# Lillthorin/YoloLite-Official-Repo

Hardware: AMD Instinct MI355X
Metric: images/sec (higher is better)
Workload: dtype f32

## Files before the change

### yololite-official-repo_amd/csrc/yl_convc.hip

```cpp
#include "yl_lp.h"
#if YL_BF16
#define yl_conv_dwc_kernel YL_LP_NAME(yl_conv_dwc_kernel)
#define yl_launch_conv_dwc YL_LP_NAME(yl_launch_conv_dwc)
#define yl_convc_init YL_LP_NAME(yl_convc_init)
#define yl_conv_pwt_kernel YL_LP_NAME(yl_conv_pwt_kernel)
#define yl_launch_conv_pwt YL_LP_NAME(yl_launch_conv_pwt)
#define yl_launch_conv_pwt_multi YL_LP_NAME(yl_launch_conv_pwt_multi)
#define yl_conv_dwt_kernel YL_LP_NAME(yl_conv_dwt_kernel)
#define yl_launch_conv_dwt YL_LP_NAME(yl_launch_conv_dwt)
#define yl_conv_dwk_kernel YL_LP_NAME(yl_conv_dwk_kernel)
#define yl_conv_dwl_kernel YL_LP_NAME(yl_conv_dwl_kernel)
#define yl_launch_conv_dwk YL_LP_NAME(yl_launch_conv_dwk)
#define yl_conv_dws_kernel YL_LP_NAME(yl_conv_dws_kernel)
#define yl_launch_conv_dws YL_LP_NAME(yl_launch_conv_dws)
#define yl_conv_wino_kernel YL_LP_NAME(yl_conv_wino_kernel)
#define yl_launch_conv_wino YL_LP_NAME(yl_launch_conv_wino)
#define yl_conv_kxk_kernel YL_LP_NAME(yl_conv_kxk_kernel)
#define yl_launch_conv_kxk YL_LP_NAME(yl_launch_conv_kxk)
#define yl_conv_pws_kernel YL_LP_NAME(yl_conv_pws_kernel)
#define yl_launch_conv_pws YL_LP_NAME(yl_launch_conv_pws)
#define yl_ir_kernel YL_LP_NAME(yl_ir_kernel)
#define yl_launch_conv_ir YL_LP_NAME(yl_launch_conv_ir)
#define yl_ir_supported YL_LP_NAME(yl_ir_supported)
#endif
// ... 1102 lines not shown

hipError_t yl_launch_conv_kxk(const YlConvP& p, hipStream_t st) {
  if (p.k != 3 || p.dw_k > 0 || (p.N & 3) || p.dec_boxes || p.C1 > 0 || p.w3p) return hipErrorNotSupported;
  static const int nwtab[4] = {0, 4, 8, -1};
  const int NWsel = nwtab[YL_DEV_KXK_NW(p.dev)];
  const int MTsel = (p.dev & YL_DEV_KXK_MT2) ? 2 : 1;
  if (p.NTtot == 4) {
    if (YlKxkLds::image_bytes(p.TK, 4) <= YlKxkLds::LIMIT || NWsel < 0) return hipErrorNotSupported;
    return NWsel == 8 ? kxk_go(p, 4, 1, 8, 1, st) : kxk_go(p, 4, 2, 4, 1, st);
  }
  if (p.NTtot % 7 != 0) return hipErrorNotSupported;
  if (YlKxkLds::image_bytes(p.TK, 7) <= YlKxkLds::LIMIT) return hipErrorNotSupported;
  const int gy = p.NTtot / 7;
  const bool eight = NWsel ? NWsel == 8 : ((long)p.M / 128) * gy >= 2 * 2 * YL_NUM_CU;
  return eight ? kxk_go(p, 7, 1, 8, gy, st) : kxk_go(p, 7, MTsel, 4, gy, st);
}

struct YlPwsLds {
  static constexpr size_t LIMIT = 64 * 1024;
  static constexpr int CH = 2;
  static constexpr __host__ __device__ size_t bytes(int NTA) { return (size_t)2 * CH * NTA * 1024; }
};

template <int NT, int NW, bool SC = false, bool DEC = false, int NT2 = 0>
__global__ __launch_bounds__(NW * 64, NW == 4 ? 3 : 4) void yl_conv_pws_kernel(YlConvP p) {
  constexpr int CH = YlPwsLds::CH;
  constexpr int NTA = NT + NT2;
  extern __shared__ __attribute__((aligned(16))) float yl_clds[];
  const int tid = threadIdx.x, lane = tid & 63;
  const int wave = __builtin_amdgcn_readfirstlane(tid >> 6);
  const int kq = lane >> 4, pl = lane & 15;
  const int KB = p.KB, NTtot = p.NTtot, Cin = p.Cin, M = p.M;
  const yl_act_t* const xin = p.x;
  f32x4* wl = reinterpret_cast<f32x4*>(yl_clds);
  const f32x4* wg = reinterpret_cast<const f32x4*>(p.wp);
  const int NC = (KB + CH - 1) / CH;
  const int G = (NTtot + NT - 1) / NT;
  const int bx = blockIdx.x, gx = gridDim.x;
  const YlBandSplit ws = yl_band_split(bx, gx, p.ntiles, G);
  const int per = ws.per, slot = ws.slot, band0 = ws.band0, bt = ws.bt, nmine = ws.nmine;
  const long total_chunks = (long)nmine * NC;
  auto load_chunk = [&](int g, int c, int buf) {
    for (int i = wave; i < CH * NTA; i += NW) {
      const int j = i / NTA, nt = i - j * NTA;
      int kb = c * CH + j;
      kb = kb < KB ? kb : KB - 1;
      if (NT2 > 0 && nt >= NT) {
        yl_glds16(reinterpret_cast<const f32x4*>(p.w3p) + ((size_t)kb * NT2 + (nt - NT)) * 64 + lane, wl + ((size_t)buf * CH * NTA + i) * 64);
        continue;
      }
      int ntg = g * NT + nt;
      ntg = ntg < NTtot ? ntg : NTtot - 1;
      yl_glds16(wg + ((size_t)kb * NTtot + ntg) * 64 + lane, wl + ((size_t)buf * CH * NTA + i) * 64);
    }
  };
  if (total_chunks > 0) load_chunk(slot / bt, 0, 0);
  long gchunk = 0;
  __syncthreads();
  const bool pre_add = (p.res || p.up) && p.act == YL_ACT_NONE;
  const float lo = yl_act_lo(p.act), hi = yl_act_hi(p.act);
  const int ohw = p.OH * p.OW;

  for (int wi = 0; wi < nmine; ++wi) {
    const int item = slot + wi * per;
    const int g = item / bt;
    const int nt0 = g * NT;
    const int tile = band0 + item - g * bt;
    YlPix px[1];
    {
      size_t lin = ((size_t)tile * NW + wave) * 16 + pl;
      px[0].valid = lin < (size_t)M;
      if (!px[0].valid) lin = (size_t)M - 1;
      px[0].lin = lin;
      px[0].b = 0; px[0].oy = 0; px[0].ox = 0;
      if (SC || DEC || p.up) {
        const int b = (int)(lin / ohw);
        const int rem = (int)(lin - (size_t)b * ohw);
        px[0].b = b;
        px[0].oy = rem / p.OW;
        px[0].ox = rem - px[0].oy * p.OW;
      }
    }
    const yl_act_t* xrow = xin + px[0].lin * Cin + 4 * kq;
    const float* srow = SC ? p.scale + (size_t)px[0].b * Cin + 4 * kq : nullptr;
    f32x4 acc[1][NTA];
#pragma unroll
    for (int nt = 0; nt < NTA; ++nt) acc[0][nt] = (f32x4){0.f, 0.f, 0.f, 0.f};
    if (pre_add) {
      const size_t obase = px[0].lin * p.N;
      size_t up_off = 0;
      if (p.up) {
        const int uy = (px[0].oy * p.UH) / p.OH, ux = (px[0].ox * p.UW) / p.OW;
        up_off = (((size_t)px[0].b * p.UH + uy) * p.UW + ux) * p.N;
      }
#pragma unroll
      for (int nt = 0; nt < NT; ++nt) {
        const int n = (nt0 + nt) * 16 + 4 * kq;
        if (n < p.N) {
          if (p.res) acc[0][nt] = yl_ld4(p.res + obase + n);
          if (p.up) acc[0][nt] += yl_ld4(p.up + up_off + n);
        }
      }
    }
    auto fetch = [&](int kb) {
      const bool ok = kb * 16 + 4 * kq < Cin;
      f32x4 v = yl_ld4(ok ? xrow + kb * 16 : p.zeros);
      if (SC) v *= yl_ld4(ok ? srow + kb * 16 : reinterpret_cast<const float*>(p.zeros));
      return v;
    };
    constexpr int PF = 4;
    f32x4 xr[PF];
#pragma unroll
    for (int i = 0; i < PF; ++i) xr[i] = fetch(i < KB ? i : KB - 1);
    auto chunk = [&](auto par, int c) {
      constexpr int P = decltype(par)::value;
      const int buf = (int)(gchunk & 1);
      if (gchunk + 1 < total_chunks) {
        if (c + 1 < NC) load_chunk(g, c + 1, buf ^ 1);
        else load_chunk((item + per) / bt, 0, buf ^ 1);
      }
      const f32x4* wb = wl + (size_t)buf * CH * NTA * 64 + lane;
#pragma unroll
      for (int j = 0; j < CH; ++j) {
        constexpr int dummy = 0; (void)dummy;
        const int kb = c * CH + j;
        if (kb < KB) {
          const int slot = (P * CH + j) % PF;
          constexpr int H0 = NTA > 7 ? (NTA + 1) / 2 : NTA;
          constexpr int H1 = NTA - H0;
          f32x4 xs[1] = {xr[slot]};
          xr[slot] = fetch(kb + PF < KB ? kb + PF : KB - 1);
          {
            f32x4 wq[H0], a0[1][H0];
#pragma unroll
            for (int nt = 0; nt < H0; ++nt) { wq[nt] = wb[(j * NTA + nt) * 64]; a0[0][nt] = acc[0][nt]; }
            yl_mma_step<H0, 1>(wq, xs, a0);
#pragma unroll
            for (int nt = 0; nt < H0; ++nt) acc[0][nt] = a0[0][nt];
          }
          if (H1 > 0) {
            constexpr int H1s = H1 > 0 ? H1 : 1;
            f32x4 wq[H1s], a1[1][H1s];
#pragma unroll
            for (int nt = 0; nt < H1; ++nt) { wq[nt] = wb[(j * NTA + H0 + nt) * 64]; a1[0][nt] = acc[0][H0 + nt]; }
            yl_mma_step<H1s, 1>(wq, xs, a1);
#pragma unroll
            for (int nt = 0; nt < H1; ++nt) acc[0][H0 + nt] = a1[0][nt];
          }
        }
      }
      __syncthreads();
      ++gchunk;
    };
    for (int c = 0; c < NC; c += 2) {
      chunk(std::integral_constant<int, 0>{}, c);
      if (c + 1 < NC) chunk(std::integral_constant<int, 1>{}, c + 1);
    }
    if (DEC) {
      if (NT2 > 0) {
        constexpr int N2 = NT2 > 0 ? NT2 : 1;
        f32x4 ad[1][NT], am[1][N2];
#pragma unroll
        for (int nt = 0; nt < NT; ++nt) ad[0][nt] = acc[0][nt];
#pragma unroll
        for (int nt = 0; nt < NT2; ++nt) am[0][nt] = acc[0][NT + nt];
        YlConvP pm = p;
        pm.bias = p.b3; pm.N = p.C3;
        yl_epi_fast<N2, 1>(pm, am, px, 0, kq, lo, hi, true);
        yl_epi_decode<NT, 1, false, true>(p, ad, px, 0, kq, lane);
      } else {
        yl_epi_decode<NT, 1, false, true>(p, *reinterpret_cast<f32x4 (*)[1][NT]>(&acc), px, 0, kq, lane);
      }
      continue;
    }
    if (!pre_add && (p.res || p.up || YL_SMOOTH(p.act))) yl_epi_generic<NTA, 1>(p, acc, px, nt0, kq);
    else yl_epi_fast<NTA, 1>(p, acc, px, nt0, kq, lo, hi, true);
  }
}

#define YL_PWS_NTS(X) X(13) X(11) X(9) X(8) X(7) X(6)
#define YL_PWS_NT_VALUE(NT) NT,
#define YL_PWS_NT_KERNELS(NT) \
  {{yl_conv_pws_kernel<NT, 4>, yl_conv_pws_kernel<NT, 4, true>}, {yl_conv_pws_kernel<NT, 8>, yl_conv_pws_kernel<NT, 8, true>}},
static const int pws_nts[6] = {YL_PWS_NTS(YL_PWS_NT_VALUE)};
static const YlConvKernel pws_kernels[6][2][2] = {YL_PWS_NTS(YL_PWS_NT_KERNELS)};
static const YlConvKernel pws_dec_kernels[2][2] = {{yl_conv_pws_kernel<6, 4, false, true>, yl_conv_pws_kernel<6, 4, false, true, 2>},
                                                   {yl_conv_pws_kernel<6, 8, false, true>, yl_conv_pws_kernel<6, 8, false, true, 2>}};

static hipError_t pws_go(const YlConvP& p0, hipStream_t st, int cand, bool eight) {
  const int NT = pws_nts[cand], NW = eight ? 8 : 4;
  YlConvP p = p0;
  p.ntiles = (int)(((long)p.M + 16 * NW - 1) / (16 * NW));
  const int gy = (p.NTtot + NT - 1) / NT;
  YlConvKernel kern = pws_kernels[cand][eight][p.scale != nullptr], asked = pws_kernels[cand][eight][0];
  int NTA = NT;
  if (p.dec_boxes) {
    if (NT != 6 || p.scale) return hipErrorNotSupported;
    kern = pws_dec_kernels[eight][p.w3p != nullptr];
    if (p.w3p) { NTA = NT + 2; asked = kern; }
  }
  const size_t lds = YlPwsLds::bytes(NTA);
  const int gx = yl_band_grid(yl_resident_blocks((const void*)asked, NW * 64, lds, 8), (long)p.ntiles * gy);
  hipLaunchKernelGGL(kern, dim3(gx), dim3(NW * 64), lds, st, p);
  return hipGetLastError();
}

hipError_t yl_launch_conv_pws(const YlConvP& p, hipStream_t st) {
  const bool dec = p.dec_boxes && !p.dec_raw;
  if (p.k != 1 || p.stride != 1 || p.dw_k > 0 || p.C1 > 0 || p.in_shift || (p.dec_boxes && !dec)) return hipErrorNotSupported;
  if (dec ? (p.NTtot != 6 || p.scale || p.res || p.up || (p.w3p && (p.C3 != 32 || YL_SMOOTH(p.act)))) : ((p.N & 3) != 0 || p.w3p)) return hipErrorNotSupported;
  if ((p.dev & YL_DEV_PWS_OFF) || p.KB < 5 || p.NTtot < 6) return hipErrorNotSupported;
  int NT = 0, cand = 0;
  double best = 1e30;
  long best_wi = 0;
  const long mt16 = ((long)p.M + 15) / 16;
  for (int i = dec ? 5 : 0; i < 6; ++i) {
    const long wi = mt16 * ((p.NTtot + pws_nts[i] - 1) / pws_nts[i]);
    const double sc = (double)((wi + 1023) / 1024) * pws_nts[i] * (wi < 1536 ? 1.25 : 1.0);
    if (sc < best) { best = sc; NT = pws_nts[i]; cand = i; best_wi = wi; }
  }
  if (best_wi < 1536) return hipErrorNotSupported;
  const int gy = (p.NTtot + NT - 1) / NT;
  const bool eight = ((long)p.M / 128) * gy >= 2 * 2 * YL_NUM_CU;
  return pws_go(p, st, cand, eight);
}

constexpr __host__ __device__ int yl_ir_pitch(int dk, int ds, int mt, int cbn) { return ((((4 * mt * cbn - 1) * ds + dk) * 16 + 7) / 64) * 64 + 56; }
constexpr __host__ __device__ int yl_ir_slab(int dk, int ds, int mt, int rbn, int cbn) { return ((4 * rbn - 1) * ds + dk) * yl_ir_pitch(dk, ds, mt, cbn); }
struct YlIrLds {
  static constexpr size_t LIMIT = 150 * 1024;
  size_t wpl, dwl, b2l, bytes;
  constexpr __host__ __device__ YlIrLds(int dk, int ds, int mt, int rbn, int cbn, int nt, int KB)
      : wpl((size_t)2 * yl_ir_slab(dk, ds, mt, rbn, cbn)), dwl(wpl + (size_t)2 * nt * 256), b2l(dwl + (size_t)KB * (dk * dk + 1) * 16),
        bytes((b2l + (size_t)KB * 16) * 4) {}
};

template <int KBI , int NT, int DK, int DS, int MT, int RBN , int CBN >
__global__ __launch_bounds__(RBN * CBN * 64, (DK == 3 && DS * MT <= 2 && KBI <= 3 && NT <= 3) ? 3 : 2) void yl_ir_kernel(YlConvP p) {
  constexpr int NWV = RBN * CBN, NTH = NWV * 64;
  constexpr int TH = 4 * RBN, TW = 4 * MT * CBN;
  constexpr int HH = (TH - 1) * DS + DK, HW = (TW - 1) * DS + DK, HN = HH * HW;
  constexpr int HMT = (HN + 15) / 16, HMW = (HMT + NWV - 1) / NWV;
  constexpr int PITCHF = yl_ir_pitch(DK, DS, MT, CBN), SLAB = yl_ir_slab(DK, DS, MT, RBN, CBN);
  extern __shared__ __attribute__((aligned(16))) float yl_clds[];
  const int tid = threadIdx.x, lane = tid & 63;
  const int wave = __builtin_amdgcn_readfirstlane(tid >> 6);
  const int kq = lane >> 4, pl = lane & 15;
  const int Cmid = p.Cin, KB = p.KB, NTtot = p.NTtot, C1 = p.C1, H = p.H, W = p.W, OH = p.OH, OW = p.OW, N = p.N;
  const YlIrLds L(DK, DS, MT, RBN, CBN, NT, KB);
  float* slab = yl_clds;
  f32x4* wpl = reinterpret_cast<f32x4*>(yl_clds + L.wpl);
  float* dwl = yl_clds + L.dwl;
  float* b2l = yl_clds + L.b2l;
  const f32x4* wg = reinterpret_cast<const f32x4*>(p.wp);
  const f32x4* w2g = reinterpret_cast<const f32x4*>(p.w2p);
  const yl_act_t* const xin = p.x;
  const yl_act_t* const up = p.up;
  {
    constexpr int T1 = DK * DK + 1;
    for (int i = tid; i < KB * T1 * 16; i += NTH) {
      const int kb = i / (T1 * 16), r = i - kb * (T1 * 16), t = r >> 4, ch = kb * 16 + (r & 15);
      dwl[i] = ch < Cmid ? (t < DK * DK ? p.dw_w[(size_t)t * Cmid + ch] : (p.dw_b ? p.dw_b[ch] : 0.0f)) : 0.0f;
    }
    for (int i = tid; i < KB * 16; i += NTH) b2l[i] = p.b2[i];
  }
  const float lo = yl_act_lo(p.act), hi = yl_act_hi(p.act);
  const float dlo = yl_act_lo(p.dw_act), dhi = yl_act_hi(p.dw_act);
  const float elo = yl_act_lo(p.act2), ehi = yl_act_hi(p.act2);
  const int dw_act = p.dw_act, act2 = p.act2;
  int h_r[HMW], h_c[HMW], h_lo[HMW];
  bool h_ok[HMW];
#pragma unroll
  for (int j = 0; j < HMW; ++j) {
    const int q = (wave + NWV * j) * 16 + pl;
    h_ok[j] = q < HN;
    const int qq = h_ok[j] ? q : 0;
    h_r[j] = qq / HW;
    h_c[j] = qq - h_r[j] * HW;
    h_lo[j] = h_r[j] * PITCHF + h_c[j] * 16 + 4 * kq;
  }
  const int rb = wave / CBN, cb = wave - rb * CBN;
  const int rbase = ((4 * rb + (pl >> 2)) * DS) * PITCHF + ((cb * 4 * MT + (pl & 3)) * DS) * 16 + 4 * kq;
  const bool pre_add = p.res != nullptr && p.act == YL_ACT_NONE;
  const int twn = OW / TW, thn = OH / TH;
  const int tiles_img = twn * thn;
  const int ntiles = p.B * tiles_img;
  int tile, tend, tstride;
  if ((gridDim.x & 7) == 0) {
    const int tpx = (ntiles + 7) >> 3;
    const int band0 = (blockIdx.x & 7) * tpx;
    tend = (band0 + tpx) < ntiles ? (band0 + tpx) : ntiles;
    tile = band0 + (blockIdx.x >> 3);
    tstride = gridDim.x >> 3;
  } else {
    tile = blockIdx.x; tend = ntiles; tstride = gridDim.x;
  }
  auto load_proj = [&](int kb, int buf) {
    for (int nt = wave; nt < NT; nt += NWV)
      yl_glds16(wg + ((size_t)kb * NTtot + (nt < NTtot ? nt : NTtot - 1)) * 64 + lane, wpl + ((size_t)buf * NT + nt) * 64);
  };
  unsigned gs = 0;
  if (tile < tend) load_proj(0, 0);
  __syncthreads();

  for (int wi = 0; tile < tend; tile += tstride, ++wi) {
    const int b = tile / tiles_img;
    const int trem = tile - b * tiles_img;
    const int tyi = trem / twn, txi = trem - tyi * twn;
    const int iy0 = tyi * TH * DS - p.dw_pad_t, ix0 = txi * TW * DS - p.dw_pad_l;
    YlPix px[MT];
#pragma unroll
    for (int mt = 0; mt < MT; ++mt) {
      px[mt].b = b;
      px[mt].oy = tyi * TH + 4 * rb + (pl >> 2);
      px[mt].ox = txi * TW + cb * 4 * MT + 4 * mt + (pl & 3);
      px[mt].valid = true;
      px[mt].lin = ((size_t)b * OH + px[mt].oy) * OW + px[mt].ox;
    }
    f32x4 xh[HMW][KBI];
    bool h_in[HMW];
    long uoff[HMW];
#pragma unroll
    for (int j = 0; j < HMW; ++j) {
      const int iy = iy0 + h_r[j], ix = ix0 + h_c[j];
      h_in[j] = h_ok[j] && iy >= 0 && iy < H && ix >= 0 && ix < W;
      uoff[j] = 0;
      if (up && h_in[j]) uoff[j] = ((((long)b * p.UH + (iy * p.UH) / H) * p.UW + (ix * p.UW) / W) * Cmid) + 4 * kq;
      const yl_act_t* src = xin + (((size_t)b * H + iy) * W + ix) * C1 + 4 * kq;
#pragma unroll
      for (int kbi = 0; kbi < KBI; ++kbi) {
        const bool ok = h_in[j] && (kbi * 16 + 4 * kq) < C1;
        xh[j][kbi] = yl_ld4(ok ? src + kbi * 16 : p.zeros);
      }
    }
    f32x4 acc[MT][NT];
#pragma unroll
    for (int mt = 0; mt < MT; ++mt)
#pragma unroll
      for (int nt = 0; nt < NT; ++nt) {
        acc[mt][nt] = (f32x4){0.f, 0.f, 0.f, 0.f};
        const int n = nt * 16 + 4 * kq;
        if (pre_add && n < N) acc[mt][nt] = yl_ld4(p.res + px[mt].lin * N + n);
      }
    f32x4 we[KBI], wn[KBI];
#pragma unroll
    for (int kbi = 0; kbi < KBI; ++kbi) wn[kbi] = w2g[((size_t)kbi * KB + 0) * 64 + lane];
    f32x4 un[HMW];
    auto load_up = [&](int kb, int j) {
      return yl_ld4((h_in[j] && kb * 16 + 4 * kq < Cmid) ? up + uoff[j] + kb * 16 : p.zeros);
    };
    if (up) {
#pragma unroll
      for (int j = 0; j < HMW; ++j) un[j] = load_up(0, j);
    }
    for (int kb = 0; kb < KB; ++kb, ++gs) {
      const int buf = (int)(gs & 1u);
#pragma unroll
      for (int kbi = 0; kbi < KBI; ++kbi) we[kbi] = wn[kbi];
      if (kb + 1 < KB) {
#pragma unroll
        for (int kbi = 0; kbi < KBI; ++kbi) wn[kbi] = w2g[((size_t)kbi * KB + kb + 1) * 64 + lane];
      }
      const f32x4 eb = yl_ld4(b2l + kb * 16 + 4 * kq);
      float* sb = slab + buf * SLAB;
#pragma unroll
      for (int j = 0; j < HMW; ++j) {
        f32x4 e[1][1] = {{{0.f, 0.f, 0.f, 0.f}}};
        if (up) e[0][0] = un[j];
#pragma unroll
        for (int kbi = 0; kbi < KBI; ++kbi) {
          const f32x4 wq1[1] = {we[kbi]};
          const f32x4 xq1[1] = {xh[j][kbi]};
          yl_mma_step<1, 1>(wq1, xq1, e);
        }
        if (up && kb + 1 < KB) un[j] = load_up(kb + 1, j);
        const f32x4 v = yl_sel4(h_in[j], yl_actc(e[0][0] + eb, act2, elo, ehi));
        if (h_ok[j]) *reinterpret_cast<f32x4*>(sb + h_lo[j]) = v;
      }
      __syncthreads();
      if (kb + 1 < KB) load_proj(kb + 1, buf ^ 1);
      else if (tile + tstride < tend) load_proj(0, buf ^ 1);
      const float* tapw = dwl + kb * ((DK * DK + 1) * 16) + 4 * kq;
      f32x4 xq[MT];
#pragma unroll
      for (int mt = 0; mt < MT; ++mt) xq[mt] = yl_ld4(tapw + DK * DK * 16);
      auto tap_row = [&](int dy) {
#pragma unroll
        for (int dx = 0; dx < DK; ++dx) {
          const f32x4 w = yl_ld4(tapw + (dy * DK + dx) * 16);
#pragma unroll
          for (int mt = 0; mt < MT; ++mt) {
            const f32x4 v = *reinterpret_cast<const f32x4*>(sb + rbase + dy * PITCHF + (dx + 4 * mt * DS) * 16);
            xq[mt].x = fmaf(v.x, w.x, xq[mt].x); xq[mt].y = fmaf(v.y, w.y, xq[mt].y);
            xq[mt].z = fmaf(v.z, w.z, xq[mt].z); xq[mt].w = fmaf(v.w, w.w, xq[mt].w);
          }
        }
      };
#pragma unroll 1
      for (int dy = 0; dy < DK; ++dy) tap_row(dy);
#pragma unroll
      for (int mt = 0; mt < MT; ++mt) xq[mt] = yl_actc(xq[mt], dw_act, dlo, dhi);
      f32x4 wq[NT];
      const f32x4* wrow = wpl + (size_t)buf * NT * 64 + lane;
#pragma unroll
      for (int nt = 0; nt < NT; ++nt) wq[nt] = wrow[nt * 64];
      yl_mma_step<NT, MT>(wq, xq, acc);
    }
    if (!pre_add && (p.res || YL_SMOOTH(p.act))) yl_epi_generic<NT, MT>(p, acc, px, 0, kq);
    else yl_epi_fast<NT, MT>(p, acc, px, 0, kq, lo, hi, true);
  }
}

template <int KBI, int NT, int DK, int DS, int MT, int RBN, int CBN>
static hipError_t ir_go(const YlConvP& p, hipStream_t st) {
  const size_t lds = YlIrLds(DK, DS, MT, RBN, CBN, NT, p.KB).bytes;
  const long ntiles = (long)p.B * (p.OH / (4 * RBN)) * (p.OW / (4 * MT * CBN));
  int gx = yl_resident_blocks((const void*)yl_ir_kernel<KBI, NT, DK, DS, MT, RBN, CBN>, RBN * CBN * 64, lds, 8);
  if (gx > ntiles) gx = (int)ntiles;
  if (gx >= 8) gx &= ~7;
  hipLaunchKernelGGL((yl_ir_kernel<KBI, NT, DK, DS, MT, RBN, CBN>), dim3(gx), dim3(RBN * CBN * 64), lds, st, p);
  return hipGetLastError();
}

#define YL_IR_SHAPES(X)                                                                                              \
  X(1, 2, 3, 2, 1, 2, 2) X(2, 2, 3, 1, 2, 2, 2) X(2, 3, 5, 2, 1, 2, 2) X(3, 3, 5, 1, 2, 2, 2) X(3, 6, 3, 2, 1, 2, 2)    \
  X(3, 3, 3, 1, 1, 2, 2) X(2, 6, 3, 1, 2, 2, 2) X(3, 6, 3, 1, 1, 2, 2)
#define YL_IR_BUCKET_LO(B) ((B) == 2 ? 0 : (B) == 3 ? 2 : (B) == 4 ? 3 : 4)

bool yl_ir_supported(int c1, int cmid, int n, int dk, int ds, int oh, int ow) {
  const int kbi = (c1 + 15) / 16, nt = (n + 15) / 16;
#define YL_IR_CHECK(A, B, C, D, E, R, S)                                                                             \
  if (kbi == A && nt <= B && nt > YL_IR_BUCKET_LO(B) && dk == C && ds == D && (oh % (4 * R)) == 0 &&                    \
      (ow % (4 * E * S)) == 0 && YlIrLds(C, D, E, R, S, B, (cmid + 15) / 16).bytes <= YlIrLds::LIMIT) return true;
  YL_IR_SHAPES(YL_IR_CHECK)
#undef YL_IR_CHECK
  return false;
}

hipError_t yl_launch_conv_ir(const YlConvP& p, hipStream_t st) {
  if (p.C1 <= 0 || p.k != 1 || p.dw_k == 0 || (p.N & 3)) return hipErrorNotSupported;
  const int kbi = (p.C1 + 15) / 16, nt = p.NTtot;
#define YL_IR_RUN(A, B, C, D, E, R, S)                                                                               \
  if (kbi == A && nt <= B && nt > YL_IR_BUCKET_LO(B) && p.dw_k == C && p.dw_stride == D && (p.OH % (4 * R)) == 0 &&     \
      (p.OW % (4 * E * S)) == 0 && YlIrLds(C, D, E, R, S, B, p.KB).bytes <= YlIrLds::LIMIT)                                 \
    return ir_go<A, B, C, D, E, R, S>(p, st);
  YL_IR_SHAPES(YL_IR_RUN)
#undef YL_IR_RUN
  return hipErrorNotSupported;
}

struct YlDwkLds {
  static constexpr size_t LIMIT = 96 * 1024;
  static constexpr __host__ __device__ int steps(int NT, int GW) { return GW == 1 ? 3 : (GW * NT <= 16 ? 2 : 1); }
  size_t dwl, bytes;
  constexpr __host__ __device__ YlDwkLds(int NT, int GW, int Cin)
      : dwl((size_t)2 * steps(NT, GW) * GW * NT * 256), bytes((dwl + yl_taps_floats(3, Cin)) * 4) {}
};

template <int NT, int GW, int NW>
__global__ __launch_bounds__(NW * 64, GW == 1 ? 3 : 2) void yl_conv_dwk_kernel(YlConvP p) {
  constexpr int S = YlDwkLds::steps(NT, GW);
  constexpr int PCS = S * GW * NT;
  extern __shared__ __attribute__((aligned(16))) float yl_clds[];
  const int tid = threadIdx.x, lane = tid & 63;
  const int wave = __builtin_amdgcn_readfirstlane(tid >> 6);
  const int kq = lane >> 4, pl = lane & 15;
  const int KB = p.KB, NTtot = p.NTtot;
  const int Cin = p.Cin, H = p.H, W = p.W, DS = p.dw_stride, pad_t = p.dw_pad_t, pad_l = p.dw_pad_l;
  const int ohw = p.OH * p.OW, OW = p.OW, M = p.M;
  const yl_act_t* const xin = p.x;
  const __amdgpu_buffer_rsrc_t xrs = __builtin_amdgcn_make_buffer_rsrc(
      const_cast<yl_act_t*>(xin), 0, (int)((long)p.B * H * W * Cin * (long)sizeof(yl_act_t)), 0x00020000);
  f32x4* wl = reinterpret_cast<f32x4*>(yl_clds);
  float* dwl = yl_clds + YlDwkLds(NT, GW, Cin).dwl;
  const f32x4* wg = reinterpret_cast<const f32x4*>(p.wp);
  const int NC = (KB + S - 1) / S;
  const int G = NTtot / (NT * GW);
  const int bx = blockIdx.x, gx = gridDim.x;
  const YlBandSplit ws = yl_band_split(bx, gx, p.ntiles, G);
  const int per = ws.per, slot = ws.slot, band0 = ws.band0, bt = ws.bt, nmine = ws.nmine;
  const long total_chunks = (long)nmine * NC;
  auto load_chunk = [&](int g, int c, int buf) {
    for (int i = wave; i < PCS; i += NW) {
      const int j = i / (GW * NT), nt = i - j * (GW * NT);
      const int kb = c * S + j;
      if (kb < KB) yl_glds16(wg + ((size_t)kb * NTtot + g * (GW * NT) + nt) * 64 + lane, wl + ((size_t)buf * PCS + i) * 64);
    }
  };
  if (total_chunks > 0) load_chunk(slot / bt, 0, 0);
  {
    const int nw = 9 * Cin;
    yl_glds_floats(p.dw_w, dwl, nw, tid, NW * 64);
    if (p.dw_b) yl_glds_floats(p.dw_b, dwl + nw, Cin, tid, NW * 64);
    else for (int i = tid; i < Cin; i += NW * 64) dwl[nw + i] = 0.0f;
  }
  long gchunk = 0;
  __syncthreads();
  const bool pre_add = (p.res || p.up) && p.act == YL_ACT_NONE;
  const float lo = yl_act_lo(p.act), hi = yl_act_hi(p.act);
  const float dlo = yl_act_lo(p.dw_act), dhi = yl_act_hi(p.dw_act);
  const int dw_act = p.dw_act;

  for (int wi = 0; wi < nmine; ++wi) {
    const int item = slot + wi * per;
    const int g = item / bt;
    const int nt0 = g * (GW * NT);
    const int tile = band0 + item - g * bt;
    YlPix px[1];
    {
      px[0] = yl_pix(((size_t)tile * NW + wave) * 16 + pl, M, ohw, OW);
    }
    f32x4 acc[GW][1][NT];
#pragma unroll
    for (int gw = 0; gw < GW; ++gw)
#pragma unroll
      for (int nt = 0; nt < NT; ++nt) acc[gw][0][nt] = (f32x4){0.f, 0.f, 0.f, 0.f};
    if (pre_add) {
      const size_t obase = px[0].lin * p.N;
      size_t up_off = 0;
      if (p.up) {
        const int uy = (px[0].oy * p.UH) / p.OH, ux = (px[0].ox * p.UW) / p.OW;
        up_off = (((size_t)px[0].b * p.UH + uy) * p.UW + ux) * p.N;
      }
#pragma unroll
      for (int gw = 0; gw < GW; ++gw)
#pragma unroll
        for (int nt = 0; nt < NT; ++nt) {
          const int n = (nt0 + gw * NT + nt) * 16 + 4 * kq;
          if (n < p.N) {
            if (p.res) acc[gw][0][nt] = yl_ld4(p.res + obase + n);
            if (p.up) acc[gw][0][nt] += yl_ld4(p.up + up_off + n);
          }
        }
    }
    unsigned tp[9];
#pragma unroll
    for (int tap = 0; tap < 9; ++tap) {
      const int iy = px[0].oy * DS - pad_t + tap / 3, ix = px[0].ox * DS - pad_l + tap % 3;
      const bool in = iy >= 0 && iy < H && ix >= 0 && ix < W;
      tp[tap] = in ? (unsigned)((((px[0].b * H + iy) * W + ix) * Cin + 4 * kq) * (int)sizeof(yl_act_t)) : 0x80000000u;
    }
    auto fetch = [&](f32x4 (&dst)[9], int kb) {
#pragma unroll
      for (int tap = 0; tap < 9; ++tap) {
#if YL_F16S
        dst[tap] = __builtin_convertvector(__builtin_bit_cast(yl_h16x4, __builtin_amdgcn_raw_buffer_load_b64(xrs, (int)tp[tap], kb * 32, 0)), f32x4);
#else
        dst[tap] = __builtin_bit_cast(f32x4, __builtin_amdgcn_raw_buffer_load_b128(xrs, (int)tp[tap], kb * 64, 0));
#endif
      }
    };
    f32x4 xt[9];
    fetch(xt, 0);
    for (int c = 0; c < NC; ++c, ++gchunk) {
      const int buf = (int)(gchunk & 1);
      if (gchunk + 1 < total_chunks) {
        if (c + 1 < NC) load_chunk(g, c + 1, buf ^ 1);
        else load_chunk((item + per) / bt, 0, buf ^ 1);
      }
      const f32x4* wb = wl + (size_t)buf * PCS * 64 + lane;
#pragma unroll
      for (int j = 0; j < S; ++j) {
        const int kb = c * S + j;
        if (kb < KB) {
          const int cc = kb * 16 + 4 * kq;
          const int cs = cc < Cin ? cc : Cin - 4;
          const float* tapw = dwl + cs;
          f32x4 xq[1];
          xq[0] = yl_ld4(tapw + 9 * Cin);
#pragma unroll
          for (int tap = 0; tap < 9; ++tap) {
            const f32x4 w = yl_ld4(tapw + tap * Cin);
            xq[0].x = fmaf(xt[tap].x, w.x, xq[0].x); xq[0].y = fmaf(xt[tap].y, w.y, xq[0].y);
            xq[0].z = fmaf(xt[tap].z, w.z, xq[0].z); xq[0].w = fmaf(xt[tap].w, w.w, xq[0].w);
          }
          xq[0] = yl_sel4(cc < Cin, yl_actc(xq[0], dw_act, dlo, dhi));
          if (kb + 1 < KB) fetch(xt, kb + 1);
#pragma unroll
          for (int gw = 0; gw < GW; ++gw) {
            f32x4 wq[NT];
#pragma unroll
            for (int nt = 0; nt < NT; ++nt) wq[nt] = wb[((j * GW + gw) * NT + nt) * 64];
            yl_mma_step<NT, 1>(wq, xq, acc[gw]);
          }
        }
      }
      __syncthreads();
    }
#pragma unroll
    for (int gw = 0; gw < GW; ++gw) {
      if (!pre_add && (p.res || p.up || YL_SMOOTH(p.act))) yl_epi_generic<NT, 1>(p, acc[gw], px, nt0 + gw * NT, kq);
      else yl_epi_fast<NT, 1>(p, acc[gw], px, nt0 + gw * NT, kq, lo, hi, true);
    }
  }
}

#define YL_DWK_SHAPES(X) X(7, 1, 4) X(7, 3, 4) X(8, 1, 4) X(8, 2, 4)
static YlConvKernel dwk_kernel_of(int NT, int GW, int NW) {
#define YL_DWK_PICK(A, B, C) if (NT == A && GW == B && NW == C) return yl_conv_dwk_kernel<A, B, C>;
  YL_DWK_SHAPES(YL_DWK_PICK)
#undef YL_DWK_PICK
  return nullptr;
}

static hipError_t dwk_go(const YlConvP& p0, hipStream_t st, int NT, int GW) {
  constexpr int NW = 4;
  const YlConvKernel kern = dwk_kernel_of(NT, GW, NW);
  if (!kern) return hipErrorNotSupported;
  YlConvP p = p0;
  p.ntiles = (int)(((long)p.M + 16 * NW - 1) / (16 * NW));
  const size_t lds = YlDwkLds(NT, GW, p.Cin).bytes;
  if (lds > YlDwkLds::LIMIT) return hipErrorNotSupported;
  const int G = p.NTtot / (NT * GW);
  const int gx = yl_band_grid(yl_resident_blocks((const void*)kern, NW * 64, lds, 8), (long)p.ntiles * G);
  hipLaunchKernelGGL(kern, dim3(gx), dim3(NW * 64), lds, st, p);
  return hipGetLastError();
}

static YlConvKernel dwl_kernel_of(int NTT);
static hipError_t dwl_go(const YlConvP& p0, hipStream_t st, YlConvKernel kern);

hipError_t yl_launch_conv_dwk(const YlConvP& p, hipStream_t st) {
  if (p.dw_k != 3 || (p.N & 3) || p.dec_boxes || p.C1 > 0 || p.KB < 12 || p.NTtot <= 8) return hipErrorNotSupported;
  if ((size_t)p.B * p.H * p.W * p.Cin * sizeof(yl_act_t) >= ((size_t)1 << 31)) return hipErrorNotSupported;
  const int sel = YL_DEV_DWK(p.dev) == 2 ? 0 : (YL_DEV_DWK(p.dev) == 1 ? 1 : 2);
  if (sel == 0) return hipErrorNotSupported;
  if (!YL_F16S && !(p.dev & YL_DEV_DWL_OFF) && p.dw_stride == 1 && p.dw_pad_t == 1 && p.dw_pad_l == 1 && !p.scale &&
      (size_t)p.B * p.H * p.W * p.Cin < ((size_t)1 << 31)) {
    const long wins = (long)p.B * ((p.OW + 7) >> 3) * ((p.OH + 7) >> 3);
    if (((long)p.B * p.OH * p.OW * 10 >= wins * 64 * 8 && wins >= 3 * YL_NUM_CU) || (p.dev & YL_DEV_DWL_ALL)) {
      if (const YlConvKernel kl = dwl_kernel_of(p.NTtot)) return dwl_go(p, st, kl);
    }
  }
  if (p.NTtot == 21) return dwk_go(p, st, 7, sel == 2 ? 3 : 1);
  if (p.NTtot == 16) return dwk_go(p, st, 8, sel == 2 ? 2 : 1);
  if (p.NTtot % 7 == 0) return dwk_go(p, st, 7, 1);
  if (p.NTtot % 8 == 0) return dwk_go(p, st, 8, 1);
  return hipErrorNotSupported;
}

struct YlDwlLds {
  static constexpr size_t LIMIT = 128 * 1024;
  static constexpr int RP = 12, RM = 512;
  int NTP;
  size_t Rl, dwl, bytes;
  constexpr __host__ __device__ YlDwlLds(int NTT, int KB)
      : NTP((NTT + 7) & ~7), Rl((size_t)3 * NTP * 64), dwl(Rl + 2 * 2 * RM), bytes(dwl * 16 + (size_t)KB * 160 * 4) {}
};

template <int NTT>
__global__ __launch_bounds__(512, 2) void yl_conv_dwl_kernel(YlConvP p) {
  constexpr YlDwlLds L(NTT, 0);
  constexpr int RP = YlDwlLds::RP, RM = YlDwlLds::RM, NTP = L.NTP;
  constexpr int NCH = NTT == 16 ? 4 : 6;
  static_assert(NTT == 16 || NTT == 21, "n-tile groups");
  auto c0of = [](int c) { return NTT == 16 ? 4 * c : (c <= 3 ? 4 * c : 12 + 3 * (c - 3)); };
  extern __shared__ __attribute__((aligned(16))) float yl_clds[];
  f32x4* const Wl = reinterpret_cast<f32x4*>(yl_clds);
  f32x4* const Rl = Wl + L.Rl;
  float* const dwl = reinterpret_cast<float*>(Wl + L.dwl);
  const int tid = threadIdx.x, lane = tid & 63;
  const int wave = __builtin_amdgcn_readfirstlane(tid >> 6);
  const int kq = lane >> 4, pl = lane & 15;
  const int KB = p.KB, NTtot = p.NTtot, Cin = p.Cin, H = p.H, W = p.W, OH = p.OH, OW = p.OW;
  const int WX = (OW + 7) >> 3, WY = (OH + 7) >> 3;
  const int wimg = WX * WY;
  const long WTOT = (long)p.B * wimg;
  const yl_act_t* const xin = p.x;
  const int wgmax = KB * NTtot - 1;
  const int bx = blockIdx.x, gx = gridDim.x;
  const YlBandSplit ws = yl_band_split(bx, gx, p.ntiles);
  const int per = ws.per, slot = ws.slot, band0 = ws.band0, band1 = ws.band1;
  const int rs = wave * 64 + lane;
  const int rP = rs >> 2, rkq = (rs & 3) ^ (((rP >> 2) & 1) << 1);
  const int ry = rP / RP, rx = rP - ry * RP;
  const bool rpix = ry < 10 && rx < 10;
  const int wsel = wave >> 2, qy = (wave >> 1) & 1, qx = wave & 1;
  const int sy = pl >> 2, sx = pl & 3;
  int ts[9];
#pragma unroll
  for (int tap = 0; tap < 9; ++tap) {
    const int P = (4 * qy + sy + tap / 3) * RP + 4 * qx + sx + tap % 3;
    ts[tap] = wsel * RM + 4 * P + (kq ^ (((P >> 2) & 1) << 1));
  }
  for (int i = tid; i < KB * 160; i += 512) {
    const int kb = i / 160, r = i - kb * 160, t = r >> 4, ch = kb * 16 + (r & 15);
    dwl[i] = ch < Cin ? (t < 9 ? p.dw_w[(size_t)t * Cin + ch] : (p.dw_b ? p.dw_b[ch] : 0.0f)) : 0.0f;
  }
  const __amdgpu_buffer_rsrc_t xrs = __builtin_amdgcn_make_buffer_rsrc(
      const_cast<yl_act_t*>(xin), 0, (int)((long)p.B * H * W * Cin * (long)sizeof(yl_act_t)), 0x00020000);
  const __amdgpu_buffer_rsrc_t wrs = __builtin_amdgcn_make_buffer_rsrc(
      const_cast<float*>(p.wp), 0, (int)((long)KB * NTtot * 1024), 0x00020000);
  constexpr unsigned OOB = 0x80000000u;
  const int lane16 = lane * 16;
  const int sh = KB & 1;
  const bool pre_add = (p.res || p.up) && p.act == YL_ACT_NONE;
  const float lo = yl_act_lo(p.act), hi = yl_act_hi(p.act);
  const float dlo = yl_act_lo(p.dw_act), dhi = yl_act_hi(p.dw_act);
  const int dw_act = p.dw_act;

  unsigned voff[2];
  auto issue_win = [&](int kb, int buf) {
#pragma unroll
    for (int w2 = 0; w2 < 2; ++w2)
      __builtin_amdgcn_raw_ptr_buffer_load_lds(xrs, (__attribute__((address_space(3))) void*)(Rl + (buf * 2 + w2) * RM + wave * 64), 16,
                                               (int)voff[w2], kb * 16 * (int)sizeof(yl_act_t), 0, 0);
  };
  auto issue_wts = [&](int kb, int wb) {
#pragma unroll
    for (int j = 0; j < NTP / 8; ++j) {
      const int i = wave + 8 * j;
      int src = kb * NTtot + (i < NTT ? i : 0);
// ... 927 lines not shown
```

Baseline: 50820.

## Software-pipeline expansion GEMM of next chunk with depthwise taps in IR kernel

Restructures the fused inverted-residual kernel so the expansion (1x1 MMA) for the next channel block, or for the next tile's first block, is computed and written to the alternate LDS slab while the depthwise taps of the current block run. The expansion work is split into per-row groups interleaved with the tap loads and FMAs using sched_barriers, and input staging, weight loads and residual preloads move one step ahead. The aim is to hide LDS and global latency and keep matrix and vector units busy at the same time. The cost is higher register pressure (tap values are held in registers, plus staged state) and more complex control flow, including an explicit waitcnt before the barrier.

```diff
diff --git a/yololite-official-repo_amd/csrc/yl_convc.hip b/yololite-official-repo_amd/csrc/yl_convc.hip
--- a/yololite-official-repo_amd/csrc/yl_convc.hip
+++ b/yololite-official-repo_amd/csrc/yl_convc.hip
@@ -1428,24 +1428,27 @@
   unsigned gs = 0;
   if (tile < tend) load_proj(0, 0);
   __syncthreads();
-
-  for (int wi = 0; tile < tend; tile += tstride, ++wi) {
-    const int b = tile / tiles_img;
-    const int trem = tile - b * tiles_img;
+  if (tile >= tend) return;
+
+  constexpr int RG = 1, NG = DK / RG;
+  f32x4 xh[HMW][KBI];
+  bool h_in[HMW];
+  long uoff[HMW];
+  f32x4 un[HMW];
+  f32x4 we[KBI], eb;
+  int etile = tile, ekb = 0;
+  auto load_up = [&](int kb, int j) __attribute__((always_inline)) {
+    return yl_ld4((h_in[j] && kb * 16 + 4 * kq < Cmid) ? up + uoff[j] + kb * 16 : p.zeros);
+  };
+  auto load_wexp = [&](int kb) __attribute__((always_inline)) {
+#pragma unroll
+    for (int kbi = 0; kbi < KBI; ++kbi) we[kbi] = w2g[((size_t)kbi * KB + kb) * 64 + lane];
+  };
+  auto stage_tile = [&](int t) __attribute__((always_inline)) {
+    const int b = t / tiles_img;
+    const int trem = t - b * tiles_img;
     const int tyi = trem / twn, txi = trem - tyi * twn;
     const int iy0 = tyi * TH * DS - p.dw_pad_t, ix0 = txi * TW * DS - p.dw_pad_l;
-    YlPix px[MT];
-#pragma unroll
-    for (int mt = 0; mt < MT; ++mt) {
-      px[mt].b = b;
-      px[mt].oy = tyi * TH + 4 * rb + (pl >> 2);
-      px[mt].ox = txi * TW + cb * 4 * MT + 4 * mt + (pl & 3);
-      px[mt].valid = true;
-      px[mt].lin = ((size_t)b * OH + px[mt].oy) * OW + px[mt].ox;
-    }
-    f32x4 xh[HMW][KBI];
-    bool h_in[HMW];
-    long uoff[HMW];
 #pragma unroll
     for (int j = 0; j < HMW; ++j) {
       const int iy = iy0 + h_r[j], ix = ix0 + h_c[j];
@@ -1459,71 +1462,120 @@
         xh[j][kbi] = yl_ld4(ok ? src + kbi * 16 : p.zeros);
       }
     }
-    f32x4 acc[MT][NT];
+    if (up) {
+#pragma unroll
+      for (int j = 0; j < HMW; ++j) un[j] = load_up(0, j);
+    }
+  };
+  f32x4 e[1][1];
+  auto e_share = [&](int g, float* sb) __attribute__((always_inline)) {
+#pragma unroll
+    for (int j = 0; j < HMW; ++j) {
+#pragma unroll
+      for (int kbi = 0; kbi < KBI; ++kbi) {
+        if ((j * KBI + kbi) * NG / (HMW * KBI) != g) continue;
+        if (kbi == 0) {
+          e[0][0] = (f32x4){0.f, 0.f, 0.f, 0.f};
+          if (up) e[0][0] = un[j];
+        }
+        const f32x4 wq1[1] = {we[kbi]};
+        const f32x4 xq1[1] = {xh[j][kbi]};
+        yl_mma_step<1, 1>(wq1, xq1, e);
+        if (kbi == KBI - 1) {
+          if (up && ekb + 1 < KB) un[j] = load_up(ekb + 1, j);
+          const f32x4 v = yl_sel4(h_in[j], yl_actc(e[0][0] + eb, act2, elo, ehi));
+          if (h_ok[j]) *reinterpret_cast<f32x4*>(sb + h_lo[j]) = v;
+        }
+      }
+    }
+  };
+  auto e_end = [&]() __attribute__((always_inline)) {
+    if (++ekb == KB) {
+      ekb = 0;
+      etile += tstride;
+      if (etile < tend) stage_tile(etile);
+    }
+    if (etile < tend) {
+      load_wexp(ekb);
+      eb = yl_ld4(b2l + ekb * 16 + 4 * kq);
+    }
+  };
+  YlPix px[MT];
+  auto set_px = [&](int t, YlPix (&q)[MT]) __attribute__((always_inline)) {
+    const int b = t / tiles_img;
+    const int trem = t - b * tiles_img;
+    const int tyi = trem / twn, txi = trem - tyi * twn;
+#pragma unroll
+    for (int mt = 0; mt < MT; ++mt) {
+      q[mt].b = b;
+      q[mt].oy = tyi * TH + 4 * rb + (pl >> 2);
+      q[mt].ox = txi * TW + cb * 4 * MT + 4 * mt + (pl & 3);
+      q[mt].valid = true;
+      q[mt].lin = ((size_t)b * OH + q[mt].oy) * OW + q[mt].ox;
+    }
+  };
+  f32x4 acc[MT][NT];
+  auto load_res = [&](const YlPix (&q)[MT], f32x4 (&r)[MT][NT]) __attribute__((always_inline)) {
 #pragma unroll
     for (int mt = 0; mt < MT; ++mt)
 #pragma unroll
       for (int nt = 0; nt < NT; ++nt) {
-        acc[mt][nt] = (f32x4){0.f, 0.f, 0.f, 0.f};
+        r[mt][nt] = (f32x4){0.f, 0.f, 0.f, 0.f};
         const int n = nt * 16 + 4 * kq;
-        if (pre_add && n < N) acc[mt][nt] = yl_ld4(p.res + px[mt].lin * N + n);
-      }
-    f32x4 we[KBI], wn[KBI];
-#pragma unroll
-    for (int kbi = 0; kbi < KBI; ++kbi) wn[kbi] = w2g[((size_t)kbi * KB + 0) * 64 + lane];
-    f32x4 un[HMW];
-    auto load_up = [&](int kb, int j) {
-      return yl_ld4((h_in[j] && kb * 16 + 4 * kq < Cmid) ? up + uoff[j] + kb * 16 : p.zeros);
-    };
-    if (up) {
-#pragma unroll
-      for (int j = 0; j < HMW; ++j) un[j] = load_up(0, j);
-    }
+        if (pre_add && n < N) r[mt][nt] = yl_ld4(p.res + q[mt].lin * N + n);
+      }
+  };
+  set_px(tile, px);
+  load_res(px, acc);
+  stage_tile(tile);
+  load_wexp(0);
+  eb = yl_ld4(b2l + 4 * kq);
+#pragma unroll
+  for (int g = 0; g < NG; ++g) e_share(g, slab);
+  e_end();
+
+  for (; tile < tend; tile += tstride) {
+    const bool more = tile + tstride < tend;
     for (int kb = 0; kb < KB; ++kb, ++gs) {
       const int buf = (int)(gs & 1u);
-#pragma unroll
-      for (int kbi = 0; kbi < KBI; ++kbi) we[kbi] = wn[kbi];
-      if (kb + 1 < KB) {
-#pragma unroll
-        for (int kbi = 0; kbi < KBI; ++kbi) wn[kbi] = w2g[((size_t)kbi * KB + kb + 1) * 64 + lane];
-      }
-      const f32x4 eb = yl_ld4(b2l + kb * 16 + 4 * kq);
-      float* sb = slab + buf * SLAB;
-#pragma unroll
-      for (int j = 0; j < HMW; ++j) {
-        f32x4 e[1][1] = {{{0.f, 0.f, 0.f, 0.f}}};
-        if (up) e[0][0] = un[j];
-#pragma unroll
-        for (int kbi = 0; kbi < KBI; ++kbi) {
-          const f32x4 wq1[1] = {we[kbi]};
-          const f32x4 xq1[1] = {xh[j][kbi]};
-          yl_mma_step<1, 1>(wq1, xq1, e);
-        }
-        if (up && kb + 1 < KB) un[j] = load_up(kb + 1, j);
-        const f32x4 v = yl_sel4(h_in[j], yl_actc(e[0][0] + eb, act2, elo, ehi));
-        if (h_ok[j]) *reinterpret_cast<f32x4*>(sb + h_lo[j]) = v;
-      }
+      const bool en = etile < tend;
+      __builtin_amdgcn_s_waitcnt(0x0F70);
       __syncthreads();
-      if (kb + 1 < KB) load_proj(kb + 1, buf ^ 1);
-      else if (tile + tstride < tend) load_proj(0, buf ^ 1);
+      if (en) load_proj(ekb, buf ^ 1);
       const float* tapw = dwl + kb * ((DK * DK + 1) * 16) + 4 * kq;
+      const float* sd = slab + buf * SLAB + rbase;
+      float* se = slab + (buf ^ 1) * SLAB;
       f32x4 xq[MT];
 #pragma unroll
       for (int mt = 0; mt < MT; ++mt) xq[mt] = yl_ld4(tapw + DK * DK * 16);
-      auto tap_row = [&](int dy) {
-#pragma unroll
-        for (int dx = 0; dx < DK; ++dx) {
-          const f32x4 w = yl_ld4(tapw + (dy * DK + dx) * 16);
+      f32x4 tw[RG * DK], tv[RG * DK][MT];
+#pragma unroll
+      for (int g = 0; g < NG; ++g) {
+#pragma unroll
+        for (int r = 0; r < RG; ++r)
+#pragma unroll
+          for (int dx = 0; dx < DK; ++dx) {
+            const int dy = g * RG + r;
+            tw[r * DK + dx] = yl_ld4(tapw + (dy * DK + dx) * 16);
+#pragma unroll
+            for (int mt = 0; mt < MT; ++mt)
+              tv[r * DK + dx][mt] = *reinterpret_cast<const f32x4*>(sd + dy * PITCHF + (dx + 4 * mt * DS) * 16);
+          }
+        __builtin_amdgcn_sched_barrier(0);
+        if (en) e_share(g, se);
+        __builtin_amdgcn_sched_barrier(0);
+#pragma unroll
+        for (int t = 0; t < RG * DK; ++t)
 #pragma unroll
           for (int mt = 0; mt < MT; ++mt) {
-            const f32x4 v = *reinterpret_cast<const f32x4*>(sb + rbase + dy * PITCHF + (dx + 4 * mt * DS) * 16);
+            const f32x4 v = tv[t][mt], w = tw[t];
             xq[mt].x = fmaf(v.x, w.x, xq[mt].x); xq[mt].y = fmaf(v.y, w.y, xq[mt].y);
             xq[mt].z = fmaf(v.z, w.z, xq[mt].z); xq[mt].w = fmaf(v.w, w.w, xq[mt].w);
           }
-        }
-      };
-#pragma unroll 1
-      for (int dy = 0; dy < DK; ++dy) tap_row(dy);
+#pragma unroll
+        for (int mt = 0; mt < MT; ++mt) asm volatile("" : "+v"(xq[mt]));
+      }
+      if (en) e_end();
 #pragma unroll
       for (int mt = 0; mt < MT; ++mt) xq[mt] = yl_actc(xq[mt], dw_act, dlo, dhi);
       f32x4 wq[NT];
@@ -1534,6 +1586,10 @@
     }
     if (!pre_add && (p.res || YL_SMOOTH(p.act))) yl_epi_generic<NT, MT>(p, acc, px, 0, kq);
     else yl_epi_fast<NT, MT>(p, acc, px, 0, kq, lo, hi, true);
+    if (more) {
+      set_px(tile + tstride, px);
+      load_res(px, acc);
+    }
   }
 }
 
```

Measured after the change: 51060 (median of 3 runs). Within noise of the previous version (+0.5%).
